# si220/Forest-SLAM

Measured on AMD Instinct MI355X. Metric: stereo frames/sec (extract+match+local-BA) at 600p, 1/8 MI355X; ATE RMSE, higher is better.
Workload: dtype mixed: u8/u16 integer (FAST, BRIEF, Hamming, SGM), f32 (ORB angle/Harris, back-projection), f64 (PnP, BA incl. its Schur GEMM on f64 MFMA); 1 GPU; stereo VO front end, configs[1]: 960x600, ORB nfeatures=1000, BF-Hamming xcheck (L+R), SGBM-3way 96 disp, back-projection, PnP-RANSAC, local BA K=10; width=960, height=600, nfeatures=1000, local_ba=window K=10 per frame, 10 LM iterations (fvo_ba_windows), parallelism=seq-per-gpu x1

## Files before the change

### forest-slam_amd/csrc/orb.hip

```cpp
#include <cmath>
#include <cstring>

#include "fvo_device.h"
#include "orb_pattern.inc"

namespace {

struct OrbDev {
  int nlevels, total_rows;
  int row0[FVO_MAX_LEVELS + 1];
  int w[FVO_MAX_LEVELS], h[FVO_MAX_LEVELS];
  long long off[FVO_MAX_LEVELS + 1];
  long long cand_off[FVO_MAX_LEVELS + 1];
  float scale[FVO_MAX_LEVELS];
  int nfeat[FVO_MAX_LEVELS];
  int tile0[FVO_MAX_LEVELS + 1];
  int ntx[FVO_MAX_LEVELS];
  int btile0[FVO_MAX_LEVELS + 1];
  int bntx[FVO_MAX_LEVELS];
};
__constant__ int c_umax[20];
__constant__ signed char c_pattern[256 * 4];

constexpr int kSelThreads = 512;
constexpr int kSelCap1 = 10000, kSelCap2 = 4096;

__device__ __forceinline__ int level_of_row(const OrbDev& G, int r) {
  int l = 0;
#pragma unroll
  for (int k = 1; k < FVO_MAX_LEVELS; ++k)
    if (k < G.nlevels && r >= G.row0[k]) l = k;
  return l;
}

__global__ void k_copy_level0(const uint8_t* __restrict__ img, int64_t stride, int pitch, uint8_t* __restrict__ pyr,
                              int64_t total, int W, int H) {
  int x = blockIdx.x * blockDim.x + threadIdx.x;
  int y = blockIdx.y;
  int b = blockIdx.z;
  if (x >= W) return;
  pyr[b * total + (int64_t)y * W + x] = img[b * stride + (int64_t)y * pitch + x];
}

__global__ void k_copy_level0_v(const uint4* __restrict__ img, int64_t stride16, int pitch16,
                                uint4* __restrict__ pyr, int64_t total16, int W16, int H, int batch) {
  const int64_t n = (int64_t)batch * H * W16;
  for (int64_t i = (int64_t)blockIdx.x * blockDim.x + threadIdx.x; i < n; i += (int64_t)gridDim.x * blockDim.x) {
    const int64_t row = i / W16;
    const int x = (int)(i - row * W16);
    const int b = (int)(row / H), y = (int)(row - (int64_t)b * H);
    pyr[b * total16 + (int64_t)y * W16 + x] = img[b * stride16 + (int64_t)y * pitch16 + x];
  }
}

constexpr int kResRows = 4, kResCols = 4;
__global__ void k_resize(const OrbDev G, uint8_t* __restrict__ pyr, int64_t total, int l, const int32_t* __restrict__ xofs,
                         const int32_t* __restrict__ xc1, const int32_t* __restrict__ yofs,
                         const int32_t* __restrict__ yc1) {
  const XcdBlock xb = xcd_block();
  const int x0 = (xb.x * blockDim.x + threadIdx.x) * kResCols;
  const int b = xb.z;
  const int w = G.w[l], h = G.h[l];
  if (x0 >= w) return;
  const int sw = G.w[l - 1], sh = G.h[l - 1];
  const uint8_t* src = pyr + b * total + G.off[l - 1];
  uint8_t* dst = pyr + b * total + G.off[l];
  int oxa[kResCols], oxb[kResCols];
  uint32_t cx0[kResCols], cx1[kResCols];
#pragma unroll
  for (int i = 0; i < kResCols; ++i) {
    const int ox = xofs[min(x0 + i, w - 1)];
    oxa[i] = ox >= 0 ? ox : (ox == -1 ? 0 : sw - 1);
    oxb[i] = ox >= 0 ? ox + 1 : oxa[i];
    cx1[i] = ox >= 0 ? (uint32_t)xc1[min(x0 + i, w - 1)] : 0u;
    cx0[i] = 256u - cx1[i];
  }
  const bool win8 = x0 + kResCols <= w && xofs[x0] >= 0 && xofs[x0 + kResCols - 1] >= 0 &&
                    oxb[kResCols - 1] - oxa[0] <= 7;
  auto window = [&](const uint8_t* row) -> uint64_t {
    const uintptr_t pa = reinterpret_cast<uintptr_t>(row + oxa[0]);
    const uint32_t* q = reinterpret_cast<const uint32_t*>(pa & ~(uintptr_t)3);
    const uint32_t sft = (uint32_t)(pa & 3);
    const uint32_t w0 = q[0], w1 = q[1], w2 = q[2];
    return ((uint64_t)__builtin_amdgcn_alignbyte(w2, w1, sft) << 32) | __builtin_amdgcn_alignbyte(w1, w0, sft);
  };
  uint32_t v[kResRows][kResCols];
#pragma unroll
  for (int k = 0; k < kResRows; ++k) {
    const int y = min(xb.y * kResRows + k, h - 1);
    const int oy = yofs[y];
    const int ra = oy >= 0 ? oy : (oy == -1 ? 0 : sh - 1), rb = oy >= 0 ? oy + 1 : ra;
    const uint32_t cy1 = oy >= 0 ? (uint32_t)yc1[y] : 0u, cy0 = 256u - cy1;
    const uint8_t* sa = src + (int64_t)ra * sw;
    const uint8_t* sb = src + (int64_t)rb * sw;
    if (win8) {
      const uint64_t wa = window(sa), wb = window(sb);
#pragma unroll
      for (int i = 0; i < kResCols; ++i) {
        const int da = 8 * (oxa[i] - oxa[0]), db = 8 * (oxb[i] - oxa[0]);
        const uint32_t ha = cx0[i] * (uint32_t)((wa >> da) & 255u) + cx1[i] * (uint32_t)((wa >> db) & 255u);
        const uint32_t hb = cx0[i] * (uint32_t)((wb >> da) & 255u) + cx1[i] * (uint32_t)((wb >> db) & 255u);
        v[k][i] = (ha * cy0 + hb * cy1 + 32768u) >> 16;
      }
    } else {
#pragma unroll
      for (int i = 0; i < kResCols; ++i) {
        const uint32_t ha = cx0[i] * sa[oxa[i]] + cx1[i] * sa[oxb[i]], hb = cx0[i] * sb[oxa[i]] + cx1[i] * sb[oxb[i]];
        v[k][i] = (ha * cy0 + hb * cy1 + 32768u) >> 16;
      }
    }
  }
#pragma unroll
  for (int k = 0; k < kResRows; ++k) {
    const int y = xb.y * kResRows + k;
#pragma unroll
    for (int i = 0; i < kResCols; ++i)
      if (y < h && x0 + i < w) dst[(int64_t)y * w + x0 + i] = (uint8_t)(v[k][i] > 255u ? 255u : v[k][i]);
  }
}

__constant__ int c_cdx[16] = {0, 1, 2, 3, 3, 3, 2, 1, 0, -1, -2, -3, -3, -3, -2, -1};
__constant__ int c_cdy[16] = {3, 3, 2, 1, 0, -1, -2, -3, -3, -3, -2, -1, 0, 1, 2, 3};

constexpr int kTW = 64, kTH = 32, kFT = 256;
static_assert(kTH <= 64 && kFT >= 2 * kTH && kFT % 64 == 0, "FAST tile shape");
constexpr int kRecKeep = 0, kRecPre = 8 * kTH, kRecSc = kRecPre + 2 * kTH;
constexpr int kTRec = kRecSc + kTH * kTW / 2;

constexpr int kFW = kTW + 2, kFH = kTH + 2;
constexpr int kPG = (kFW + 3) / 4;
constexpr int kIC = 4, kIW = kTW + 12, kIH = kTH + 8;

typedef unsigned short u16x2 __attribute__((ext_vector_type(2)));
__device__ __forceinline__ u16x2 as_u16x2(uint32_t v) { return __builtin_bit_cast(u16x2, v); }
__device__ __forceinline__ uint32_t as_u32(u16x2 v) { return __builtin_bit_cast(uint32_t, v); }
__device__ __forceinline__ u16x2 bytes02(uint32_t v) { return as_u16x2(__builtin_amdgcn_perm(0u, v, 0x0c020c00u)); }
__device__ __forceinline__ u16x2 bytes13(uint32_t v) { return as_u16x2(__builtin_amdgcn_perm(0u, v, 0x0c030c01u)); }

__device__ __forceinline__ u16x2 two_of_four(u16x2 a, u16x2 b, u16x2 c, u16x2 d) {
  const u16x2 lab = __builtin_elementwise_min(a, b), hab = __builtin_elementwise_max(a, b);
  const u16x2 lcd = __builtin_elementwise_min(c, d), hcd = __builtin_elementwise_max(c, d);
  return __builtin_elementwise_max(__builtin_elementwise_max(lab, lcd), __builtin_elementwise_min(hab, hcd));
}
__device__ __forceinline__ uint32_t fast_pre2(u16x2 v, u16x2 p0, u16x2 p4, u16x2 p8, u16x2 p12, u16x2 t) {
  const u16x2 vt = v + t, vm = __builtin_elementwise_sub_sat(v, t);
  auto br = [&](u16x2 p) { return __builtin_elementwise_sub_sat(p, vt); };
  auto dk = [&](u16x2 p) { return __builtin_elementwise_sub_sat(vm, p); };
  return as_u32(__builtin_elementwise_max(two_of_four(br(p0), br(p4), br(p8), br(p12)),
                                          two_of_four(dk(p0), dk(p4), dk(p8), dk(p12))));
}

__device__ __forceinline__ bool has9(unsigned m) {
  const unsigned mm = m | (m << 16);
  const unsigned c2 = mm & (mm >> 1), c4 = c2 & (c2 >> 2), c8 = c4 & (c4 >> 4), c9 = c8 & (c8 >> 1);
  return (c9 & 0xFFFFu) != 0;
}

__device__ __forceinline__ int tile_level(const OrbDev& G, int t) {
  int l = 0;
#pragma unroll
  for (int k = 1; k < FVO_MAX_LEVELS; ++k)
    if (k < G.nlevels && t >= G.tile0[k]) l = k;
  return l;
}

template <bool SCOREMAP>
__global__ __launch_bounds__(kFT) void k_fast_nms(const OrbDev G, const uint8_t* __restrict__ pyr,
                                                  uint8_t* __restrict__ score, uint8_t* __restrict__ trec,
                                                  int64_t total, int thr, int edge, int org, int ntiles) {
  __shared__ __attribute__((aligned(16))) uint8_t s_img[kIH][kIW];
  __shared__ __attribute__((aligned(16))) uint8_t s_sc[kFH][kFW];
  __shared__ uint16_t s_list[kFH * kFW];
  __shared__ uint16_t s_pre[kFH * kPG * 4];
  __shared__ uint32_t s_m[kTH][2];
  __shared__ int s_rp[kTH];
  __shared__ int s_n, s_npre;
  const XcdBlock xb = xcd_block();
  const int b = xb.y, t = xb.x;
  const int l = tile_level(G, t);
  const int lt = t - G.tile0[l];
  const int tx = lt % G.ntx[l], ty = lt / G.ntx[l];
  const int x0 = org + tx * kTW, y0 = org + ty * kTH;
  const int w = G.w[l], h = G.h[l];
  const uint8_t* im = pyr + b * total + G.off[l];
  if (x0 >= 8 && x0 + kTW + 12 <= w && y0 >= 4 && y0 + kTH + 4 <= h) {
    for (int i = threadIdx.x; i < kIH * (kIW / 4); i += kFT) {
      const int r = i / (kIW / 4), k = i % (kIW / 4);
      const uint8_t* p = im + (int64_t)(y0 - 4 + r) * w + x0 - 1 - kIC + 4 * k;
      const uint32_t* a = reinterpret_cast<const uint32_t*>(reinterpret_cast<uintptr_t>(p) & ~(uintptr_t)3);
      const uint32_t sh = (uint32_t)(reinterpret_cast<uintptr_t>(p) & 3);
      *reinterpret_cast<uint32_t*>(&s_img[r][4 * k]) = __builtin_amdgcn_alignbyte(a[1], a[0], sh);
    }
  } else {
    for (int i = threadIdx.x; i < kIH * kIW; i += kFT) {
      const int r = i / kIW, c = i % kIW;
      const int y = min(max(y0 - 4 + r, 0), h - 1), x = min(max(x0 - 1 - kIC + c, 0), w - 1);
      s_img[r][c] = im[(int64_t)y * w + x];
    }
  }
  for (int i = threadIdx.x; i < kFH * kFW / 4; i += kFT) reinterpret_cast<uint32_t*>(&s_sc[0][0])[i] = 0;
  if (threadIdx.x < 2 * kTH) (&s_m[0][0])[threadIdx.x] = 0u;
  if (threadIdx.x == 0) { s_n = 0; s_npre = 0; }
  __syncthreads();
  const u16x2 tt = {(unsigned short)thr, (unsigned short)thr};
  for (int i0 = 0; i0 < kFH * kPG; i0 += kFT) {
    const int i = i0 + threadIdx.x;
    const int r = i / kPG, g = i % kPG;
    const int y = y0 - 1 + r, xg = x0 - 1 + 4 * g;
    unsigned f = 0;
    if (i < kFH * kPG && y >= 3 && y < h - 3) {
      const uint32_t* rc = reinterpret_cast<const uint32_t*>(&s_img[r + 3][0]);
      const uint32_t dv = rc[g + 1];
      const uint32_t d0 = reinterpret_cast<const uint32_t*>(&s_img[r + 6][0])[g + 1];
      const uint32_t d8 = reinterpret_cast<const uint32_t*>(&s_img[r][0])[g + 1];
      const uint32_t d4 = __builtin_amdgcn_alignbyte(rc[g + 2], dv, 3);
      const uint32_t d12 = __builtin_amdgcn_alignbyte(dv, rc[g], 1);
      const uint32_t e = fast_pre2(bytes02(dv), bytes02(d0), bytes02(d4), bytes02(d8), bytes02(d12), tt);
      const uint32_t o = fast_pre2(bytes13(dv), bytes13(d0), bytes13(d4), bytes13(d8), bytes13(d12), tt);
      f = (unsigned)((e & 0xFFFFu) != 0) | (unsigned)((o & 0xFFFFu) != 0) << 1 | (unsigned)((e >> 16) != 0) << 2 |
          (unsigned)((o >> 16) != 0) << 3;
      const int lo = max(3 - xg, 0), hi = min(min(w - 3 - xg, kFW - 4 * g), 4);
      f &= hi > lo ? ((1u << hi) - 1u) & ~((1u << lo) - 1u) : 0u;
    }
    const unsigned long long m0 = __ballot(f & 1u), m1 = __ballot(f & 2u), m2 = __ballot(f & 4u),
                             m3 = __ballot(f & 8u);
    const int lane = threadIdx.x & 63;
    const unsigned long long below = (1ull << lane) - 1ull;
    int pos = __popcll(m0 & below) + __popcll(m1 & below) + __popcll(m2 & below) + __popcll(m3 & below);
    int base = 0;
    const int tot = __popcll(m0) + __popcll(m1) + __popcll(m2) + __popcll(m3);
    if (lane == 0 && tot) base = atomicAdd(&s_npre, tot);
    pos += __shfl(base, 0, 64);
    const int ib = r * kFW + 4 * g;
#pragma unroll
    for (int j = 0; j < 4; ++j)
      if ((f >> j) & 1u) s_pre[pos++] = (uint16_t)(ib + j);
  }
  __syncthreads();
  const int npre = s_npre;
  for (int j0 = 0; j0 < npre; j0 += kFT) {
    const int j = j0 + threadIdx.x;
    bool corner = false;
    int i = 0;
    if (j < npre) {
      i = s_pre[j];
      const int r = i / kFW, c = i % kFW;
      const int v = s_img[r + 3][c + kIC];
      const u16x2 vt = {(unsigned short)(v + thr), (unsigned short)(v + thr)};
      const u16x2 vm = {(unsigned short)(v - thr), (unsigned short)(v - thr)};
      uint32_t ab = 0, ad = 0;
#pragma unroll
      for (int k = 0; k < 8; ++k) {
        const uint32_t pk = (uint32_t)s_img[r + 3 + c_cdy[k]][c + kIC + c_cdx[k]] |
                            (uint32_t)s_img[r + 3 + c_cdy[k + 8]][c + kIC + c_cdx[k + 8]] << 16;
        const u16x2 sh = {(unsigned short)(15 - k), (unsigned short)(15 - k)};
        const uint32_t K = 0x10001u << k;
        ab |= as_u32((vt - as_u16x2(pk)) >> sh) & K;
        ad |= as_u32((as_u16x2(pk) - vm) >> sh) & K;
      }
      const unsigned bright = __builtin_amdgcn_perm(0u, ab, 0x0c0c0200u);
      const unsigned dark = __builtin_amdgcn_perm(0u, ad, 0x0c0c0200u);
      corner = has9(bright) || has9(dark);
    }
    const unsigned long long m = __ballot(corner);
    int base = 0;
    if ((threadIdx.x & 63) == 0 && m) base = atomicAdd(&s_n, __popcll(m));
    base = __shfl(base, 0, 64);
    if (corner) s_list[base + __popcll(m & ((1ull << (threadIdx.x & 63)) - 1ull))] = (uint16_t)i;
  }
  __syncthreads();
// ... 774 lines not shown
    g.scale[l] = s;
    g.w[l] = cv_round_f((float)c.width * inv);
    g.h[l] = cv_round_f((float)c.height * inv);
    g.off[l] = off;
    off += (int64_t)g.w[l] * g.h[l];
    g.row0[l] = row;
    row += g.h[l];
    int rw = std::max(g.w[l] - 2 * c.edge_threshold, 0), rh = std::max(g.h[l] - 2 * c.edge_threshold, 0);
    g.cand_off[l] = coff;
    coff += (int64_t)((rw + 1) / 2) * ((rh + 1) / 2) + 1;
  }
  g.off[c.nlevels] = off;
  g.row0[c.nlevels] = row;
  g.cand_off[c.nlevels] = coff;
  g.total_px = (off + 255) / 256 * 256;
  g.total_rows = row;
  g.cand_total = coff;
  {
    float factor = (float)(1.0 / sf);
    float nd = c.nfeatures * (1 - factor) / (1 - (float)std::pow((double)factor, (double)c.nlevels));
    int sum = 0;
    for (int l = 0; l < c.nlevels - 1; ++l) {
      g.nfeat[l] = cv_round_f(nd);
      sum += g.nfeat[l];
      nd *= factor;
    }
    g.nfeat[c.nlevels - 1] = std::max(c.nfeatures - sum, 0);
  }

  std::vector<int32_t> xo, xc, yo, yc;
  auto coeffs = [](int src, int dst, std::vector<int32_t>& ofs, std::vector<int32_t>& c1) {
    double inv_scale = (double)dst / (double)src;
    double scale = 1.0 / inv_scale;
    for (int d = 0; d < dst; ++d) {
      double fval = scale * ((double)d + 0.5) - 0.5;
      int ival = (int)std::floor(fval);
      if (ival >= 0 && src > 1) {
        if (ival < src - 1) {
          double frac = fval - (double)ival;
          ofs.push_back(ival);
          c1.push_back(frac < 0 ? 0 : (int)std::llrint(frac * 256.0));
        } else {
          ofs.push_back(-2);
          c1.push_back(0);
        }
      } else {
        ofs.push_back(-1);
        c1.push_back(0);
      }
    }
  };
  for (int l = 1; l < c.nlevels; ++l) {
    ctx->rt.xoff[l] = (int64_t)xo.size();
    coeffs(g.w[l - 1], g.w[l], xo, xc);
    ctx->rt.yoff[l] = (int64_t)yo.size();
    coeffs(g.h[l - 1], g.h[l], yo, yc);
  }
  if (xo.empty()) { xo.push_back(0); xc.push_back(0); yo.push_back(0); yc.push_back(0); }
  int rc = 0;
  if ((rc = fvo_alloc(ctx, &ctx->rt.xofs, xo.size())) || (rc = fvo_alloc(ctx, &ctx->rt.xc1, xc.size())) ||
      (rc = fvo_alloc(ctx, &ctx->rt.yofs, yo.size())) || (rc = fvo_alloc(ctx, &ctx->rt.yc1, yc.size())))
    return rc;
  FVO_HIP(ctx, hipMemcpy(ctx->rt.xofs, xo.data(), xo.size() * 4, hipMemcpyHostToDevice));
  FVO_HIP(ctx, hipMemcpy(ctx->rt.xc1, xc.data(), xc.size() * 4, hipMemcpyHostToDevice));
  FVO_HIP(ctx, hipMemcpy(ctx->rt.yofs, yo.data(), yo.size() * 4, hipMemcpyHostToDevice));
  FVO_HIP(ctx, hipMemcpy(ctx->rt.yc1, yc.data(), yc.size() * 4, hipMemcpyHostToDevice));

  int half = c.patch_size / 2;
  std::vector<int> umax(half + 2 > 20 ? half + 2 : 20, 0);
  int vmax = (int)std::floor(half * std::sqrt(2.f) / 2 + 1);
  int vmin = (int)std::ceil(half * std::sqrt(2.f) / 2);
  for (int v = 0; v <= vmax; ++v) umax[v] = (int)std::lrint(std::sqrt((double)half * half - v * v));
  for (int v = half, v0 = 0; v >= vmin; --v) {
    while (umax[v0] == umax[v0 + 1]) ++v0;
    umax[v] = v0;
    ++v0;
  }

  g.angle_pass = half > kAngR || c.edge_threshold < half;

  FVO_HIP(ctx, hipMemcpyToSymbol(HIP_SYMBOL(c_umax), umax.data(), sizeof(int) * 20));
  FVO_HIP(ctx, hipMemcpyToSymbol(HIP_SYMBOL(c_pattern), FVO_ORB_PATTERN, sizeof(FVO_ORB_PATTERN)));

  const int64_t B = c.max_batch;
  int64_t maxcand = 0;
  for (int l = 0; l < c.nlevels; ++l) maxcand = std::max<int64_t>(maxcand, g.cand_off[l + 1] - g.cand_off[l]);
  ctx->scratch_per = 2 * maxcand;
  if ((rc = fvo_alloc(ctx, &ctx->pyr, B * g.total_px)) ||
      (rc = fvo_alloc(ctx, &ctx->cand, B * g.cand_total)) ||
      (rc = fvo_alloc(ctx, &ctx->hel, B * g.cand_total)) || (rc = fvo_alloc(ctx, &ctx->ncand, B * c.nlevels)) ||
      (rc = fvo_alloc(ctx, &ctx->nsel1, B * c.nlevels)) || (rc = fvo_alloc(ctx, &ctx->nsel2, B * c.nlevels)) ||
      (rc = fvo_alloc(ctx, &ctx->koff, B * (c.nlevels + 1))) ||
      (rc = fvo_alloc(ctx, &ctx->scratch, B * c.nlevels * ctx->scratch_per)))
    return rc;
  if ((rc = fvo_alloc(ctx, &ctx->fast_rec, B * make_dev(g, c.edge_threshold).tile0[g.nlevels] * kTRec))) return rc;
  return 0;
}

namespace {
OrbDev make_dev(const OrbGeom& g, int org) {
  OrbDev G{};
  G.nlevels = g.nlevels;
  G.total_rows = g.total_rows;
  int t = 0, bt = 0;
  for (int l = 0; l < g.nlevels; ++l) {
    G.row0[l] = g.row0[l];
    G.w[l] = g.w[l];
    G.h[l] = g.h[l];
    G.off[l] = g.off[l];
    G.cand_off[l] = g.cand_off[l];
    G.scale[l] = g.scale[l];
    G.nfeat[l] = g.nfeat[l];
    const int ew = g.w[l] - 2 * org, eh = g.h[l] - 2 * org;
    G.ntx[l] = ew > 0 && eh > 0 ? (ew + kTW - 1) / kTW : 0;
    G.tile0[l] = t;
    t += G.ntx[l] ? G.ntx[l] * ((eh + kTH - 1) / kTH) : 0;
    G.bntx[l] = (g.w[l] + kBW - 1) / kBW;
    G.btile0[l] = bt;
    bt += G.bntx[l] * ((g.h[l] + kBH - 1) / kBH);
  }
  G.btile0[g.nlevels] = bt;
  G.row0[g.nlevels] = g.row0[g.nlevels];
  G.off[g.nlevels] = g.off[g.nlevels];
  G.cand_off[g.nlevels] = g.cand_off[g.nlevels];
  G.tile0[g.nlevels] = t;
  return G;
}
}

int orb_run(fvo_ctx* ctx, const uint8_t* images, int batch, int64_t image_stride, int pitch, float* kp, uint8_t* desc,
            int32_t* counts, int cap, hipStream_t s) {
  const fvo_config& c = ctx->cfg;
  const OrbGeom& g = ctx->g;
  const int L = g.nlevels;
  const int W = c.width, H = c.height;
  const int64_t total = g.total_px;
  const int thr = std::min(std::max(c.fast_threshold, 0), 255);
  const OrbDev G = make_dev(g, c.edge_threshold);
  const int ntiles = G.tile0[L];
  const bool vec = ((uintptr_t)images & 15) == 0 && (image_stride & 15) == 0 && (pitch & 15) == 0 && (W & 15) == 0 &&
                   (total & 15) == 0;
  if (vec) {
    const int64_t n16 = (int64_t)batch * H * (W / 16);
    const int nblk = (int)std::min<int64_t>((n16 + 255) / 256, 4096);
    FVO_TIMED(ctx, KN_ORB_COPY, s, hipLaunchKernelGGL(k_copy_level0_v, dim3(nblk), dim3(256), 0, s,
                                                      reinterpret_cast<const uint4*>(images), image_stride / 16,
                                                      pitch / 16, reinterpret_cast<uint4*>(ctx->pyr), total / 16, W / 16,
                                                      H, batch));
  } else {
    FVO_TIMED(ctx, KN_ORB_COPY, s, hipLaunchKernelGGL(k_copy_level0, dim3((W + 255) / 256, H, batch), dim3(256), 0, s,
                                                      images, image_stride, pitch, ctx->pyr, total, W, H));
  }
  for (int l = 1; l < L; ++l)
    FVO_TIMED(ctx, KN_ORB_RESIZE, s, hipLaunchKernelGGL(k_resize, dim3((g.w[l] + 256 * kResCols - 1) / (256 * kResCols), (g.h[l] + kResRows - 1) / kResRows, batch), dim3(256), 0, s, G, ctx->pyr, total, l,
                       ctx->rt.xofs + ctx->rt.xoff[l], ctx->rt.xc1 + ctx->rt.xoff[l], ctx->rt.yofs + ctx->rt.yoff[l],
                       ctx->rt.yc1 + ctx->rt.yoff[l]));
  if (ntiles > 0)
    FVO_TIMED(ctx, KN_ORB_FAST, s, hipLaunchKernelGGL(k_fast_nms<false>, dim3(ntiles, batch), dim3(kFT), 0, s, G, ctx->pyr,
                       nullptr, ctx->fast_rec, total, thr, c.edge_threshold, c.edge_threshold, ntiles));
  FVO_TIMED(ctx, KN_ORB_SELECT1, s, hipLaunchKernelGGL(HIP_KERNEL_NAME(k_select<ElemFast, kSelCap1, true>), dim3(batch, L),
                     dim3(kSelThreads), 0, s, G, ctx->fast_rec, ntiles, c.edge_threshold, ctx->cand, ctx->ncand,
                     ctx->nsel1, ctx->scratch, ctx->scratch_per, g.cand_total, L, 2));
  FVO_TIMED(ctx, KN_ORB_HARRIS, s, hipLaunchKernelGGL(k_harris, dim3(32, L, batch), dim3(256), 0, s, G, ctx->pyr, ctx->cand, ctx->nsel1, ctx->hel, total,
                     g.cand_total, L));
  FVO_TIMED(ctx, KN_ORB_SELECT2, s, hipLaunchKernelGGL(HIP_KERNEL_NAME(k_select<ElemHarris, kSelCap2, false>), dim3(batch, L),
                     dim3(kSelThreads), 0, s, G, nullptr, ntiles, c.edge_threshold, ctx->hel, ctx->nsel1,
                     ctx->nsel2, ctx->scratch, ctx->scratch_per, g.cand_total, L, 1));
  FVO_TIMED(ctx, KN_ORB_OFFSETS, s, hipLaunchKernelGGL(k_offsets, dim3((batch + 63) / 64), dim3(64), 0, s, ctx->nsel2, ctx->koff, counts, batch, L, cap));
  if (g.angle_pass) {
    FVO_TIMED(ctx, KN_ORB_ANGLE, s, hipLaunchKernelGGL(k_angle, dim3(16, L, batch), dim3(256), 0, s, G, ctx->pyr, ctx->hel, ctx->nsel2, ctx->koff, kp,
                       total, g.cand_total, L, cap, c.patch_size));
    FVO_TIMED(ctx, KN_ORB_BRIEF, s, hipLaunchKernelGGL(k_brief<false>, dim3(64, batch), dim3(256), 0, s, G, ctx->pyr, ctx->hel, ctx->koff, kp, counts,
                       desc, total, g.cand_total, L, cap, c.patch_size));
  } else {
    FVO_TIMED(ctx, KN_ORB_BRIEF, s, hipLaunchKernelGGL(k_brief<true>, dim3(64, batch), dim3(256), 0, s, G, ctx->pyr, ctx->hel, ctx->koff, kp, counts,
                       desc, total, g.cand_total, L, cap, c.patch_size));
  }
  ctx->orb_last_batch = batch;
  FVO_LAUNCH_CHECK(ctx);
  return 0;
}

int orb_blur_debug(fvo_ctx* ctx) {
  const OrbGeom& g = ctx->g;
  if (!ctx->blur) {
    int rc = fvo_alloc(ctx, &ctx->blur, (int64_t)ctx->cfg.max_batch * g.total_px);
    if (rc) return rc;
  }
  if (ctx->orb_last_batch > 0) {
    const OrbDev G = make_dev(g, 0);
    hipLaunchKernelGGL(k_blur, dim3(G.btile0[g.nlevels], ctx->orb_last_batch), dim3(256), 0, 0, G, ctx->pyr, ctx->blur,
                       g.total_px);
    FVO_LAUNCH_CHECK(ctx);
  }
  FVO_HIP(ctx, hipDeviceSynchronize());
  return 0;
}

int orb_score_debug(fvo_ctx* ctx) {
  const OrbGeom& g = ctx->g;
  if (!ctx->score) {
    int rc = fvo_alloc(ctx, &ctx->score, (int64_t)ctx->cfg.max_batch * g.total_px);
    if (rc) return rc;
  }
  if (ctx->orb_last_batch > 0) {
    const OrbDev G = make_dev(g, 0);
    const int ntiles = G.tile0[g.nlevels];
    hipLaunchKernelGGL(k_fast_nms<true>, dim3(ntiles, ctx->orb_last_batch), dim3(kFT), 0, 0, G, ctx->pyr, ctx->score,
                       nullptr, g.total_px, std::min(std::max(ctx->cfg.fast_threshold, 0), 255),
                       ctx->cfg.edge_threshold, 0, ntiles);
    FVO_LAUNCH_CHECK(ctx);
  }
  FVO_HIP(ctx, hipDeviceSynchronize());
  return 0;
}

namespace {
__global__ void k_pack_keys(const float* __restrict__ k, uint64_t* __restrict__ a, int n) {
  int i = blockIdx.x * blockDim.x + threadIdx.x;
  if (i < n) a[i] = ((uint64_t)__float_as_uint(k[i]) << 32) | (uint32_t)i;
}
__global__ void k_unpack_idx(const uint64_t* __restrict__ a, int32_t* __restrict__ idx, int n) {
  int i = blockIdx.x * blockDim.x + threadIdx.x;
  if (i < n) idx[i] = (int32_t)(uint32_t)a[i];
}
__global__ __launch_bounds__(kSelThreads) void k_select_test(uint64_t* __restrict__ a, int n, int keep,
                                                             int32_t* __restrict__ scratch, int32_t* __restrict__ out_n) {
  __shared__ SelShared sh;
  int r = select_block<ElemHarris>(sh, a, n, keep, scratch, scratch + n);
  if (threadIdx.x == 0) *out_n = r;
}
}

int orb_retain_best_run(fvo_ctx* ctx, const float* keys, int n, int keep, int32_t* idx_out, int32_t* n_out,
                         hipStream_t s) {
  uint64_t* a = nullptr;
  int32_t* scr = nullptr;
  FVO_HIP(ctx, hipMallocAsync((void**)&a, sizeof(uint64_t) * (size_t)std::max(n, 1), s));
  FVO_HIP(ctx, hipMallocAsync((void**)&scr, sizeof(int32_t) * 2 * (size_t)std::max(n, 1), s));
  hipLaunchKernelGGL(k_pack_keys, dim3((n + 255) / 256 + 1), dim3(256), 0, s, keys, a, n);
  hipLaunchKernelGGL(k_select_test, dim3(1), dim3(kSelThreads), 0, s, a, n, keep, scr, n_out);
  hipLaunchKernelGGL(k_unpack_idx, dim3((n + 255) / 256 + 1), dim3(256), 0, s, a, idx_out, n);
  FVO_HIP(ctx, hipFreeAsync(a, s));
  FVO_HIP(ctx, hipFreeAsync(scr, s));
  FVO_LAUNCH_CHECK(ctx);
  return 0;
}
```

### forest-slam_amd/csrc/sgbm.hip

```cpp
#include <algorithm>
#include <cstdlib>
#include <type_traits>

#include "fvo_device.h"
#include "sgbm_params.h"

namespace {

typedef unsigned short u16x2 __attribute__((ext_vector_type(2)));

__device__ __forceinline__ u16x2 as_v(uint32_t x) { return __builtin_bit_cast(u16x2, x); }
__device__ __forceinline__ uint32_t as_u(u16x2 v) { return __builtin_bit_cast(uint32_t, v); }
__device__ __forceinline__ u16x2 vmin(u16x2 a, u16x2 b) { return __builtin_elementwise_min(a, b); }
__device__ __forceinline__ u16x2 splat(uint32_t s) { return as_v((s & 0xFFFFu) | (s << 16)); }
__device__ __forceinline__ u16x2 splat_p2(uint32_t m, uint32_t P2) { return as_v(__umul24(m, 0x10001u) + P2 * 0x10001u); }

constexpr uint32_t kSent = 0x7FFFu;

constexpr int kQPrev = 0x90;
constexpr int kQNext = 0xF9;
constexpr int kQX1 = 0xB1;
constexpr int kQX2 = 0x4E;

template <int CTRL>
// ... 742 lines not shown
  if constexpr (!S2) return;

  const int nseg = (W1 + SEG - 1) / SEG;
  uint32_t Rst[PQ];
  uint32_t minR = 0;
#pragma unroll
  for (int k = 0; k < PQ; ++k) Rst[k] = 0;
  uint32_t Vn[SEG][PQ], Pn[SEG][PQ], Mn[SEG], ckn[CKW];
  auto ldck = [&](int sg) {
    const int slot = SEG * (sg + 1) > W1 - 1 ? nck - 1 : sg;
    const uint32_t* cp = ckptr(slot);
#pragma unroll
    for (int kk = 0; kk < CKW; kk += 4) {
      const uint4 w4 = *reinterpret_cast<const uint4*>(cp + kk);
      ckn[kk] = w4.x; ckn[kk + 1] = w4.y; ckn[kk + 2] = w4.z; ckn[kk + 3] = w4.w;
    }
  };
  auto ldcol = [&](int sg, int i) {
    const int xx = max(W1 - 1 - (SEG * sg + i), 0);
    ld(xx, Vn[i]);
    ldp(xx, Pn[i]);
    Mn[i] = ldm(xx);
  };
  auto ldseg = [&](int sg) {
    ldck(sg);
#pragma unroll
    for (int i = SEG - 1; i >= 0; --i) ldcol(sg, i);
  };
  ldseg(0);
  auto ihi_of = [&](int sg) { return min(SEG - 1, W1 - 1 - SEG * sg); };
  uint32_t wk = 0, wn = 0;
  auto wta = [&](int i, const uint32_t* Sw) {
    uint32_t kmin = 0;
#pragma unroll
    for (int kk = 0; kk < PQ; ++kk) {
      const uint32_t jj = (uint32_t)(2 * kk) | ((uint32_t)(2 * kk + 1) << 8);
      const uint32_t klo = __builtin_amdgcn_perm(Sw[kk], jj, 0x0c050400u);
      const uint32_t khi = __builtin_amdgcn_perm(Sw[kk], jj, 0x0c070601u);
      kmin = kk == 0 ? min(klo, khi) : min(kmin, min(klo, khi));
    }
    kmin += (uint32_t)(q * DQ);
    kmin = dmin<kQX1>(kmin);
    kmin = dmin<kQX2>(kmin);
    kmin = dmin<kRHalfMirror>(kmin);
    kmin = dmin<kRMirror>(kmin);
    const int d = (int)(kmin & 0xFFu);
    uint32_t* sw = reinterpret_cast<uint32_t*>(&s_S[r][q * DQ]);
#pragma unroll
    for (int kk = 0; kk < PQ; ++kk) sw[kk] = Sw[kk];
    asm volatile("" ::: "memory");
    const uint32_t nb = ((uint32_t)s_S[r][max(d - 1, 0)] << 16) | s_S[r][min(d + 1, D - 1)];
    asm volatile("" ::: "memory");
    wk = q == i ? kmin : wk;
    wn = q == i ? nb : wn;
  };
  auto segment = [&](int sg, auto full_t) {
    constexpr bool FULL = decltype(full_t)::value;
    if constexpr (FULL) {
      uint32_t lst[PQ], Cs[SEG][PQ], part[SEG][PQ];
#pragma unroll
      for (int kk = 0; kk < PQ; ++kk) lst[kk] = ckn[kk];
      uint32_t lmin = ckn[PQ];
      ldck(sg + 1);
#pragma unroll
      for (int t = 0; t < SEG; ++t) {
        const int a = SEG - 1 - t, c = t;
        if (t < SEG / 2) {
          derive16<PQ>(Pn[a], Vn[a], Cs[a], Mn[a], P1, p.P2, q);
          derive16<PQ>(Pn[c], Vn[c], Cs[c], Mn[c], P1, p.P2, q);
        }
        lmin = step16<PQ>(lst, Cs[a], q, P1, lmin, p.P2);
        minR = step16<PQ>(Rst, Cs[c], q, P1, minR, p.P2);
        if (t < SEG / 2) {
#pragma unroll
          for (int kk = 0; kk < PQ; ++kk) {
            part[a][kk] = as_u(as_v(lst[kk]) + as_v(Vn[a][kk]));
            part[c][kk] = as_u(as_v(Rst[kk]) + as_v(Vn[c][kk]));
          }
        } else {
          uint32_t Sa[PQ], Sc[PQ];
#pragma unroll
          for (int kk = 0; kk < PQ; ++kk) {
            Sa[kk] = as_u(as_v(part[a][kk]) + as_v(lst[kk]));
            Sc[kk] = as_u(as_v(part[c][kk]) + as_v(Rst[kk]));
          }
          wta(a, Sa);
          wta(c, Sc);
          const int u = t - SEG / 2;
          ldcol(sg + 1, SEG - 1 - u);
          ldcol(sg + 1, u);
        }
      }
    } else {
      uint32_t lst[PQ], Ls[SEG][PQ], Cs[SEG][PQ];
      const bool zero = SEG * (sg + 1) > W1 - 1;
#pragma unroll
      for (int kk = 0; kk < PQ; ++kk) lst[kk] = zero ? 0u : ckn[kk];
      uint32_t lmin = zero ? 0u : ckn[PQ];
#pragma unroll
      for (int i = SEG - 1; i >= 0; --i) {
        derive16<PQ>(Pn[i], Vn[i], Cs[i], Mn[i], P1, p.P2, q);
        if (i <= ihi_of(sg)) lmin = step16<PQ>(lst, Cs[i], q, P1, lmin, p.P2);
#pragma unroll
        for (int kk = 0; kk < PQ; ++kk) Ls[i][kk] = as_u(as_v(lst[kk]) + as_v(Vn[i][kk]));
      }
#pragma unroll
      for (int i = 0; i < SEG; ++i) {
        if (i > ihi_of(sg)) break;
        minR = step16<PQ>(Rst, Cs[i], q, P1, minR, p.P2);
        uint32_t Sw[PQ];
#pragma unroll
        for (int kk = 0; kk < PQ; ++kk) Sw[kk] = as_u(as_v(Ls[i][kk]) + as_v(Rst[kk]));
        wta(i, Sw);
      }
    }
    {
      const int ihi = FULL ? SEG - 1 : ihi_of(sg);
      {
        const bool colv = q < SEG && q <= ihi;
        const int x1 = W1 - 1 - (SEG * sg + q);
        if (colv) key[(x1 + p.minX1 - p.minD - (D - 1)) & (RK - 1)] = 0xFFFFFFFFu;
        if (colv) {
          const int best = (int)(wk >> 8), d = (int)(wk & 0xFFu);
          const int sm1 = (int)(wn >> 16), sp1 = (int)(wn & 0xFFFFu);
          const int x2 = x1 + p.minX1 - d - p.minD;
          if (x2 >= 0 && x2 < W && best < 0x7FFF)
            atomicMin(&key[x2 & (RK - 1)], ((uint32_t)best << 16) | (uint32_t)(0xFFFF - x1));
          int dd;
          if (0 < d && d < D - 1) {
            const int denom2 = max(sm1 + sp1 - 2 * best, 1);
            dd = d * 16 + ((sm1 - sp1) * 16 + denom2) / (denom2 * 2);
          } else {
            dd = d * 16;
          }
          sraw[x1 & (RS - 1)] = (int16_t)(dd + p.minD * 16);
        }
      }
      const int x1_lo = W1 - 1 - (SEG * sg + ihi);
      {
        const int cnt = ihi >= 0 ? min(next_chk - (x1_lo + D) + 1, SEG) : 0;
        const bool act = q < cnt && rowok;
        const int d1 = checked(next_chk - q);
        *(act ? out + (next_chk - q + p.minX1) : sink) = (int16_t)d1;
        if (cnt > 0) next_chk -= cnt;
      }
    }
  };
#pragma unroll 1
  for (int sg = 0; sg < nseg - 1; ++sg) segment(sg, std::true_type{});
  segment(nseg - 1, std::false_type{});
  for (int x1 = next_chk - q; x1 >= 0; x1 -= 16) check(x1);
}

__global__ void k_sg_median(const int16_t* __restrict__ raw, int16_t* __restrict__ out, int W, int H,
                            const uint32_t* __restrict__ fail, int16_t invalid, int32_t* __restrict__ status) {
  const int x = blockIdx.x * blockDim.x + threadIdx.x, y = blockIdx.y, b = blockIdx.z;
  if (status && x == 0 && y == 0) status[b] = (fail && fail[b]) ? FVO_SGBM_HANDOFF_TIMEOUT : FVO_SGBM_OK;
  if (x >= W) return;
  const int16_t* s = raw + (int64_t)b * W * H;
  int v[9];
  int k = 0;
#pragma unroll
  for (int dy = -1; dy <= 1; ++dy)
#pragma unroll
    for (int dx = -1; dx <= 1; ++dx) {
      const int yy = min(max(y + dy, 0), H - 1), xx = min(max(x + dx, 0), W - 1);
      v[k++] = s[(int64_t)yy * W + xx];
    }
#define SG_S(a, b) { int t_ = min(v[a], v[b]); v[b] = max(v[a], v[b]); v[a] = t_; }
  SG_S(1, 2) SG_S(4, 5) SG_S(7, 8) SG_S(0, 1) SG_S(3, 4) SG_S(6, 7) SG_S(1, 2) SG_S(4, 5) SG_S(7, 8)
  SG_S(0, 3) SG_S(5, 8) SG_S(4, 7) SG_S(3, 6) SG_S(1, 4) SG_S(2, 5) SG_S(4, 7) SG_S(4, 2) SG_S(6, 4)
  SG_S(4, 2)
#undef SG_S
  out[((int64_t)b * H + y) * W + x] = (fail && fail[b]) ? invalid : (int16_t)v[4];
}

__global__ void k_sg_prep(uint32_t* ctl, int nb) {
  const int t = threadIdx.x;
  if (t == 0) {
    ctl[0] = 0;
    const uint32_t g = ctl[1] + 1;
    ctl[1] = g >= (1u << 25) ? 1u : g;
  }
  for (int b = t; b < nb; b += blockDim.x) ctl[4 + b] = 0;
}

int sg_nck(const SgParams& p) { return p.width1 / 8 + 2; }
int sg_ckw(int D) { return D / 32 + 1 <= 4 ? 4 : 8; }
int sg_nblk(const SgParams& p) { return (p.H + 3) / 4; }

template <int D>
void launch_sgbm(fvo_ctx* ctx, const SgParams& p, const uint8_t* L, const uint8_t* R, int nb, int64_t stride,
                 int pitch, int16_t* disp, int32_t* status, hipStream_t s) {
  uint16_t* V = ctx->sg_V;
  uint16_t* M = ctx->sg_M;
  const int nck = sg_nck(p);
  const int16_t invalid = (int16_t)((p.minD - 1) * 16);
  const fvo_config& cfg = ctx->cfg;
  if (cfg.sgbm_mode == FVO_SGBM_CLASSIC) {
    const int g = sg_lanes(cfg), cbr = sg_cols(cfg);
    typedef void (*CostKernel)(const uint8_t*, const uint8_t*, int64_t, int, SgParams, uint16_t*, uint16_t*, SgLink);
    CostKernel kern;
    int gg, cb;
    if (g == 16) kern = k_sg_costvert<D, 32, 16, false>, gg = 16, cb = 32;
    else if (g == 4 && cbr == 32) kern = k_sg_costvert<D, 32, 4, false>, gg = 4, cb = 32;
    else if (g == 4) kern = k_sg_costvert<D, 64, 4, false>, gg = 4, cb = 64;
    else if (cbr == 16) kern = k_sg_costvert<D, 16, 8, false>, gg = 8, cb = 16;
    else kern = k_sg_costvert<D, 32, 8, false>, gg = 8, cb = 32;
    const dim3 gcv((p.width1 + cb - 1) / cb, p.nstripes, nb);
    const SgLink lk{};
    FVO_TIMED(ctx, KN_SG_VERT, s, hipLaunchKernelGGL(kern, gcv, dim3(gg * cb), 0, s, L, R, stride, pitch, p, V, M, lk));
    FVO_TIMED(ctx, KN_SG_ROWS, s, hipLaunchKernelGGL(HIP_KERNEL_NAME(k_sg_rows<D, kSwBoth>), dim3(sg_nblk(p), nb), dim3(64), 0, s,
                                                     V, M, p, ctx->sg_ckpt, nck, ctx->sg_raw));
    FVO_TIMED(ctx, KN_SG_MEDIAN, s, hipLaunchKernelGGL(k_sg_median, dim3((p.W + 255) / 256, p.H, nb), dim3(256), 0, s,
                                                       ctx->sg_raw, disp, p.W, p.H, nullptr, invalid, status));
    return;
  }
  const int nk = sg_nk(p);
  const int64_t us = cfg.sgbm_handoff_us > 0 ? cfg.sgbm_handoff_us : 250000;
  const SgLink lk{ctx->sg_ckpt, nck, nk, ctx->sg_hand, ctx->sg_ctl, (uint64_t)us * 100u, cfg.sgbm_handoff_us < 0 ? 1 : 0};
  hipLaunchKernelGGL(k_sg_prep, dim3(1), dim3(256), 0, s, ctx->sg_ctl, nb);
  FVO_TIMED(ctx, KN_SG_VERT, s, hipLaunchKernelGGL(HIP_KERNEL_NAME(k_sg_costvert<D, kSgCB, 8, true>),
                                                   dim3(nk * p.nstripes * nb), dim3(8 * kSgCB), 0, s, L, R, stride, pitch,
                                                   p, V, M, lk));
  FVO_TIMED(ctx, KN_SG_ROWS, s, hipLaunchKernelGGL(HIP_KERNEL_NAME(k_sg_rows<D, kSwRight>), dim3(sg_nblk(p), nb), dim3(64), 0, s,
                                                   V, M, p, ctx->sg_ckpt, nck, ctx->sg_raw));
  FVO_TIMED(ctx, KN_SG_MEDIAN, s, hipLaunchKernelGGL(k_sg_median, dim3((p.W + 255) / 256, p.H, nb), dim3(256), 0, s,
                                                     ctx->sg_raw, disp, p.W, p.H, ctx->sg_ctl + 4, invalid, status));
}

}

int sgbm_init(fvo_ctx* ctx) {
  const fvo_config& c = ctx->cfg;
  SgParams p = make_params(c);
  const int64_t B = c.sgbm_max_batch > 0 ? std::min(c.sgbm_max_batch, c.max_batch) : c.max_batch;
  const int64_t plane = (int64_t)p.width1 * p.D;
  int rc;
  const int64_t vol = (int64_t)(p.HG4 + p.nstripes) * 4 * plane;
  const int64_t ckp = (int64_t)sg_nblk(p) * sg_nck(p) * 64 * sg_ckw(p.D);
  const int64_t hand = (int64_t)p.H * 2 * (p.D / 32) * 16;
  if ((rc = fvo_alloc(ctx, &ctx->sg_V, B * vol)) || (rc = fvo_alloc(ctx, &ctx->sg_M, B * vol / p.D)) ||
      (rc = fvo_alloc(ctx, &ctx->sg_ckpt, B * ckp)) ||
      (rc = fvo_alloc(ctx, &ctx->sg_raw, B * p.H * p.W)) || (rc = fvo_alloc(ctx, &ctx->sg_hand, B * hand)) ||
      (rc = fvo_alloc(ctx, &ctx->sg_ctl, 4 + B)))
    return rc;
  FVO_HIP(ctx, hipMemset(ctx->sg_hand, 0, B * hand * sizeof(uint64_t)));
  FVO_HIP(ctx, hipMemset(ctx->sg_ctl, 0, (4 + B) * sizeof(uint32_t)));
  return 0;
}

int sgbm_run(fvo_ctx* ctx, const uint8_t* L, const uint8_t* R, int batch, int64_t image_stride, int pitch,
             int16_t* disp, int32_t* status, hipStream_t s) {
  SgParams p = make_params(ctx->cfg);
  switch (p.D) {
    case 64: launch_sgbm<64>(ctx, p, L, R, batch, image_stride, pitch, disp, status, s); break;
    case 96: launch_sgbm<96>(ctx, p, L, R, batch, image_stride, pitch, disp, status, s); break;
    default: launch_sgbm<128>(ctx, p, L, R, batch, image_stride, pitch, disp, status, s); break;
  }
  FVO_LAUNCH_CHECK(ctx);
  return 0;
}
```

Before: 5914 frames/s.

## Tile pyramid resize through LDS and vectorize SGBM 3x3 median

The ORB pyramid resize now stages each 128x64 output tile's source window into LDS with 16-byte loads. It computes horizontal taps with perm+udot2, reuses the horizontal result when consecutive output rows share a source row, and writes dword-packed outputs using a lane shuffle. It falls back to the old direct path when the tile's source window does not fit. Separately, the SGBM median filter now handles 8 columns by 4 rows per thread using packed 16-bit min/max and 16-byte loads and stores, sharing the column sorts between rows. Both changes aim to cut per-pixel memory traffic and instruction count, at the cost of more complex alignment and edge handling.

New measurement: 5974 frames/s (median of 6 runs). 1.01x the previous value.

```diff
diff --git a/forest-slam_amd/csrc/orb.hip b/forest-slam_amd/csrc/orb.hip
--- a/forest-slam_amd/csrc/orb.hip
+++ b/forest-slam_amd/csrc/orb.hip
@@ -53,18 +53,12 @@
   }
 }
 
-constexpr int kResRows = 4, kResCols = 4;
-__global__ void k_resize(const OrbDev G, uint8_t* __restrict__ pyr, int64_t total, int l, const int32_t* __restrict__ xofs,
-                         const int32_t* __restrict__ xc1, const int32_t* __restrict__ yofs,
-                         const int32_t* __restrict__ yc1) {
-  const XcdBlock xb = xcd_block();
-  const int x0 = (xb.x * blockDim.x + threadIdx.x) * kResCols;
-  const int b = xb.z;
-  const int w = G.w[l], h = G.h[l];
+constexpr int kResCols = 4;
+__device__ __forceinline__ void resize_direct(const uint8_t* __restrict__ src, uint8_t* __restrict__ dst, int w, int h,
+                                              int sw, int sh, int x0, int y0, int rows, const int32_t* __restrict__ xofs,
+                                              const int32_t* __restrict__ xc1, const int32_t* __restrict__ yofs,
+                                              const int32_t* __restrict__ yc1) {
   if (x0 >= w) return;
-  const int sw = G.w[l - 1], sh = G.h[l - 1];
-  const uint8_t* src = pyr + b * total + G.off[l - 1];
-  uint8_t* dst = pyr + b * total + G.off[l];
   int oxa[kResCols], oxb[kResCols];
   uint32_t cx0[kResCols], cx1[kResCols];
 #pragma unroll
@@ -84,10 +78,9 @@
     const uint32_t w0 = q[0], w1 = q[1], w2 = q[2];
     return ((uint64_t)__builtin_amdgcn_alignbyte(w2, w1, sft) << 32) | __builtin_amdgcn_alignbyte(w1, w0, sft);
   };
-  uint32_t v[kResRows][kResCols];
-#pragma unroll
-  for (int k = 0; k < kResRows; ++k) {
-    const int y = min(xb.y * kResRows + k, h - 1);
+#pragma unroll 1
+  for (int y = y0; y < min(y0 + rows, h); ++y) {
+    uint32_t v[kResCols];
     const int oy = yofs[y];
     const int ra = oy >= 0 ? oy : (oy == -1 ? 0 : sh - 1), rb = oy >= 0 ? oy + 1 : ra;
     const uint32_t cy1 = oy >= 0 ? (uint32_t)yc1[y] : 0u, cy0 = 256u - cy1;
@@ -100,22 +93,142 @@
         const int da = 8 * (oxa[i] - oxa[0]), db = 8 * (oxb[i] - oxa[0]);
         const uint32_t ha = cx0[i] * (uint32_t)((wa >> da) & 255u) + cx1[i] * (uint32_t)((wa >> db) & 255u);
         const uint32_t hb = cx0[i] * (uint32_t)((wb >> da) & 255u) + cx1[i] * (uint32_t)((wb >> db) & 255u);
-        v[k][i] = (ha * cy0 + hb * cy1 + 32768u) >> 16;
+        v[i] = (ha * cy0 + hb * cy1 + 32768u) >> 16;
       }
     } else {
 #pragma unroll
       for (int i = 0; i < kResCols; ++i) {
         const uint32_t ha = cx0[i] * sa[oxa[i]] + cx1[i] * sa[oxb[i]], hb = cx0[i] * sb[oxa[i]] + cx1[i] * sb[oxb[i]];
-        v[k][i] = (ha * cy0 + hb * cy1 + 32768u) >> 16;
-      }
-    }
-  }
-#pragma unroll
-  for (int k = 0; k < kResRows; ++k) {
-    const int y = xb.y * kResRows + k;
+        v[i] = (ha * cy0 + hb * cy1 + 32768u) >> 16;
+      }
+    }
 #pragma unroll
     for (int i = 0; i < kResCols; ++i)
-      if (y < h && x0 + i < w) dst[(int64_t)y * w + x0 + i] = (uint8_t)(v[k][i] > 255u ? 255u : v[k][i]);
+      if (x0 + i < w) dst[(int64_t)y * w + x0 + i] = (uint8_t)(v[i] > 255u ? 255u : v[i]);
+  }
+}
+
+constexpr int kRzTW = 128, kRzTH = 64, kRzSR = 8;
+constexpr int kRzLds = 1024;
+static_assert(kRzTW == 32 * kResCols && kRzTH == 8 * kRzSR, "resize tile shape");
+__global__ __launch_bounds__(256) void k_resize(const OrbDev G, uint8_t* __restrict__ pyr, int64_t total, int l,
+                                                const int32_t* __restrict__ xofs, const int32_t* __restrict__ xc1,
+                                                const int32_t* __restrict__ yofs, const int32_t* __restrict__ yc1) {
+  __shared__ uint4 s_src[kRzLds + 1];
+  const int tid = threadIdx.x, cg = tid & 31, strip = tid >> 5;
+  const int tx0 = blockIdx.x * kRzTW, ty0 = blockIdx.y * kRzTH, b = blockIdx.z;
+  const int w = G.w[l], h = G.h[l], sw = G.w[l - 1], sh = G.h[l - 1];
+  uint8_t* img = pyr + b * total;
+  const int tw = min(kRzTW, w - tx0), th = min(kRzTH, h - ty0);
+  auto first = [](int o, int n) { return o >= 0 ? o : (o == -1 ? 0 : n - 1); };
+  auto last = [](int o, int n) { return o >= 0 ? o + 1 : (o == -1 ? 0 : n - 1); };
+  const int c0 = first(xofs[tx0], sw), c1 = last(xofs[tx0 + tw - 1], sw);
+  const int r0 = first(yofs[ty0], sh), r1 = last(yofs[ty0 + th - 1], sh);
+  const int ncols = c1 - c0 + 1, nrows = r1 - r0 + 1;
+  const int pitch16 = (ncols + 15 + 15) >> 4;
+  const int x0 = tx0 + cg * kResCols;
+  int wofs = 0, span = 0;
+  uint32_t sel[kResCols], cxw[kResCols];
+#pragma unroll
+  for (int i = 0; i < kResCols; ++i) {
+    const int x = min(x0 + i, w - 1);
+    const int ox = xofs[x], oa = first(ox, sw), ob = last(ox, sw);
+    const uint32_t c = ox >= 0 ? (uint32_t)xc1[x] : 0u;
+    if (i == 0) wofs = oa;
+    span = ob - wofs;
+    sel[i] = 0x0c000c00u | (uint32_t)(oa - wofs) | ((uint32_t)(ob - wofs) << 16);
+    cxw[i] = (256u - c) | (c << 16);
+  }
+  if (!__syncthreads_and(span <= 7) || pitch16 * nrows > kRzLds) {
+    resize_direct(img + G.off[l - 1], img + G.off[l], w, h, sw, sh, x0, ty0 + strip * kRzSR, kRzSR, xofs, xc1, yofs, yc1);
+    return;
+  }
+  wofs -= c0;
+
+  uint32_t rinfo[kRzSR];
+#pragma unroll
+  for (int k = 0; k < kRzSR; ++k) {
+    const int yc = min(ty0 + strip * kRzSR + k, h - 1), oy = yofs[yc];
+    rinfo[k] = (uint32_t)(first(oy, sh) - r0) | ((uint32_t)(last(oy, sh) - first(oy, sh)) << 10) |
+               ((oy >= 0 ? (uint32_t)yc1[yc] : 0u) << 16);
+  }
+  const int64_t g0 = G.off[l - 1] + (int64_t)r0 * sw + c0;
+  uint4 stage[kRzLds / 256];
+#pragma unroll
+  for (int k = 0; k < kRzLds / 256; ++k) {
+    const int i = tid + 256 * k, rr = i / pitch16, j = i - rr * pitch16;
+    const int64_t ga = g0 + (int64_t)rr * sw;
+    const int nblk = (((int)ga & 15) + ncols + 15) >> 4;
+    const bool ok = rr < nrows && j < nblk;
+    stage[k] = reinterpret_cast<const uint4*>(img + ((ok ? ga : g0) & ~(int64_t)15))[ok ? j : 0];
+  }
+#pragma unroll
+  for (int k = 0; k < kRzLds / 256; ++k)
+    if (tid + 256 * k < nrows * pitch16) s_src[tid + 256 * k] = stage[k];
+  __syncthreads();
+
+  typedef unsigned short us2 __attribute__((ext_vector_type(2)));
+  const uint32_t* lds = reinterpret_cast<const uint32_t*>(s_src);
+  const int g0lo = (int)g0 & 15;
+  auto hrow = [&](int rr, uint32_t (&hv)[kResCols]) {
+    const uint32_t p = (uint32_t)(rr * pitch16 * 16 + ((g0lo + rr * sw) & 15) + wofs);
+    const uint32_t* q = lds + (p >> 2);
+    const uint32_t w0 = q[0], w1 = q[1], w2 = q[2], sft = p & 3;
+    const uint32_t lo = __builtin_amdgcn_alignbyte(w1, w0, sft), hi = __builtin_amdgcn_alignbyte(w2, w1, sft);
+#pragma unroll
+    for (int i = 0; i < kResCols; ++i)
+      hv[i] = __builtin_amdgcn_udot2(__builtin_bit_cast(us2, __builtin_amdgcn_perm(hi, lo, sel[i])),
+                                     __builtin_bit_cast(us2, cxw[i]), 0u, false);
+  };
+  uint8_t* dst = img + G.off[l] + tx0;
+  uint32_t hp[kResCols] = {};
+  int prb = -1;
+#pragma unroll
+  for (int k = 0; k < kRzSR; ++k) {
+    const int y = ty0 + strip * kRzSR + k;
+    const int ra = (int)(rinfo[k] & 1023u), rb = ra + (int)((rinfo[k] >> 10) & 1u);
+    const uint32_t cy = rinfo[k] >> 16, cyw = (256u - cy) | (cy << 16);
+    uint32_t ha[kResCols], hb[kResCols], acc[kResCols];
+    if (ra == prb) {
+#pragma unroll
+      for (int i = 0; i < kResCols; ++i) ha[i] = hp[i];
+    } else {
+      hrow(ra, ha);
+    }
+    if (rb == ra) {
+#pragma unroll
+      for (int i = 0; i < kResCols; ++i) hb[i] = ha[i];
+    } else {
+      hrow(rb, hb);
+    }
+    prb = rb;
+#pragma unroll
+    for (int i = 0; i < kResCols; ++i) {
+      hp[i] = hb[i];
+      acc[i] = min(__builtin_amdgcn_udot2(__builtin_bit_cast(us2, ha[i] | (hb[i] << 16)), __builtin_bit_cast(us2, cyw),
+                                          32768u, false), 0xFFFFFFu);
+    }
+    const uint32_t own = __builtin_amdgcn_perm(__builtin_amdgcn_perm(acc[3], acc[2], 0x0c0c0602u),
+                                               __builtin_amdgcn_perm(acc[1], acc[0], 0x0c0c0602u), 0x05040100u);
+    const uint32_t prev = __shfl_up(own, 1, 32);
+    const int a = (int)((G.off[l] + (int64_t)y * w + tx0) & 3);
+    const uint32_t dw = (uint32_t)((((uint64_t)own << 32) | prev) >> (8 * (4 - a)));
+    if (y < h) {
+      uint8_t* row = dst + (int64_t)y * w;
+      const int cd = cg * kResCols - a;
+      if (cd >= 0 && cd + 3 < tw) {
+        *reinterpret_cast<uint32_t*>(row + cd) = dw;
+      } else {
+#pragma unroll
+        for (int j = 0; j < 4; ++j)
+          if (cd + j >= 0 && cd + j < tw) row[cd + j] = (uint8_t)(dw >> (8 * j));
+      }
+      if (cg == 31) {
+#pragma unroll
+        for (int j = 0; j < 3; ++j)
+          if (j < a && cd + 4 + j < tw) row[cd + 4 + j] = (uint8_t)(own >> (8 * (4 - a + j)));
+      }
+    }
   }
 }
 
@@ -1196,7 +1309,7 @@
                                                       images, image_stride, pitch, ctx->pyr, total, W, H));
   }
   for (int l = 1; l < L; ++l)
-    FVO_TIMED(ctx, KN_ORB_RESIZE, s, hipLaunchKernelGGL(k_resize, dim3((g.w[l] + 256 * kResCols - 1) / (256 * kResCols), (g.h[l] + kResRows - 1) / kResRows, batch), dim3(256), 0, s, G, ctx->pyr, total, l,
+    FVO_TIMED(ctx, KN_ORB_RESIZE, s, hipLaunchKernelGGL(k_resize, dim3((g.w[l] + kRzTW - 1) / kRzTW, (g.h[l] + kRzTH - 1) / kRzTH, batch), dim3(256), 0, s, G, ctx->pyr, total, l,
                        ctx->rt.xofs + ctx->rt.xoff[l], ctx->rt.xc1 + ctx->rt.xoff[l], ctx->rt.yofs + ctx->rt.yoff[l],
                        ctx->rt.yc1 + ctx->rt.yoff[l]));
   if (ntiles > 0)
diff --git a/forest-slam_amd/csrc/sgbm.hip b/forest-slam_amd/csrc/sgbm.hip
--- a/forest-slam_amd/csrc/sgbm.hip
+++ b/forest-slam_amd/csrc/sgbm.hip
@@ -918,9 +918,66 @@
   for (int x1 = next_chk - q; x1 >= 0; x1 -= 16) check(x1);
 }
 
-__global__ void k_sg_median(const int16_t* __restrict__ raw, int16_t* __restrict__ out, int W, int H,
-                            const uint32_t* __restrict__ fail, int16_t invalid, int32_t* __restrict__ status) {
-  const int x = blockIdx.x * blockDim.x + threadIdx.x, y = blockIdx.y, b = blockIdx.z;
+typedef short sg_s2 __attribute__((ext_vector_type(2)));
+constexpr int kMedRows = 4;
+__host__ __device__ inline bool sg_median_vec(const void* raw, const void* out, int W) {
+  return W % 8 == 0 && (((uintptr_t)raw | (uintptr_t)out) & 15) == 0;
+}
+inline dim3 sg_median_grid(const void* raw, const void* out, int W, int H, int nb) {
+  if (sg_median_vec(raw, out, W)) return dim3(((W / 8) * ((H + kMedRows - 1) / kMedRows) + 255) / 256, 1, nb);
+  return dim3((W + 255) / 256, H, nb);
+}
+
+#define SG_PK(a, b) { const sg_s2 t_ = __builtin_elementwise_min(a, b); b = __builtin_elementwise_max(a, b); a = t_; }
+__device__ __forceinline__ void sg_median_rows8(const int16_t* __restrict__ s, int16_t* __restrict__ o, int W, int H,
+                                                int x0, int y0, bool bad, int16_t invalid) {
+  sg_s2 t[kMedRows + 2][4][3];
+#pragma unroll
+  for (int k = 0; k < kMedRows + 2; ++k) {
+    const int16_t* row = s + (int64_t)min(max(y0 - 1 + k, 0), H - 1) * W;
+    const uint4 c4 = *reinterpret_cast<const uint4*>(row + x0);
+    const uint32_t c[4] = {c4.x, c4.y, c4.z, c4.w};
+    const uint32_t l = (uint16_t)row[max(x0 - 1, 0)], r = (uint16_t)row[min(x0 + 8, W - 1)];
+#pragma unroll
+    for (int j = 0; j < 4; ++j) {
+      const uint32_t lo = j ? (c[j - 1] >> 16) | (c[j] << 16) : l | (c[0] << 16);
+      const uint32_t hi = j < 3 ? (c[j] >> 16) | (c[j + 1] << 16) : (c[3] >> 16) | (r << 16);
+      sg_s2 a = __builtin_bit_cast(sg_s2, lo), m = __builtin_bit_cast(sg_s2, c[j]), z = __builtin_bit_cast(sg_s2, hi);
+      SG_PK(m, z) SG_PK(a, m) SG_PK(m, z)
+      t[k][j][0] = a, t[k][j][1] = m, t[k][j][2] = z;
+    }
+  }
+  const uint32_t inv2 = (uint16_t)invalid * 0x10001u;
+#pragma unroll
+  for (int k = 0; k < kMedRows; ++k) {
+    uint32_t res[4];
+#pragma unroll
+    for (int j = 0; j < 4; ++j) {
+      sg_s2 v0 = t[k][j][0], v1 = t[k][j][1], v2 = t[k][j][2], v3 = t[k + 1][j][0], v4 = t[k + 1][j][1],
+            v5 = t[k + 1][j][2], v6 = t[k + 2][j][0], v7 = t[k + 2][j][1], v8 = t[k + 2][j][2];
+      SG_PK(v0, v3) SG_PK(v5, v8) SG_PK(v4, v7) SG_PK(v3, v6) SG_PK(v1, v4) SG_PK(v2, v5) SG_PK(v4, v7) SG_PK(v4, v2)
+      SG_PK(v6, v4) SG_PK(v4, v2)
+      res[j] = bad ? inv2 : __builtin_bit_cast(uint32_t, v4);
+    }
+    if (y0 + k < H) *reinterpret_cast<uint4*>(o + (int64_t)(y0 + k) * W + x0) = make_uint4(res[0], res[1], res[2], res[3]);
+  }
+}
+#undef SG_PK
+
+__global__ __launch_bounds__(256) void k_sg_median(const int16_t* __restrict__ raw, int16_t* __restrict__ out, int W, int H,
+                                                   const uint32_t* __restrict__ fail, int16_t invalid,
+                                                   int32_t* __restrict__ status) {
+  const int b = blockIdx.z;
+  if (sg_median_vec(raw, out, W)) {
+    const int W8 = W >> 3, i = blockIdx.x * blockDim.x + threadIdx.x;
+    const bool bad = fail && fail[b];
+    if (status && i == 0) status[b] = bad ? FVO_SGBM_HANDOFF_TIMEOUT : FVO_SGBM_OK;
+    const int yg = i / W8;
+    if (yg * kMedRows >= H) return;
+    sg_median_rows8(raw + (int64_t)b * W * H, out + (int64_t)b * W * H, W, H, (i - yg * W8) * 8, yg * kMedRows, bad, invalid);
+    return;
+  }
+  const int x = blockIdx.x * blockDim.x + threadIdx.x, y = blockIdx.y;
   if (status && x == 0 && y == 0) status[b] = (fail && fail[b]) ? FVO_SGBM_HANDOFF_TIMEOUT : FVO_SGBM_OK;
   if (x >= W) return;
   const int16_t* s = raw + (int64_t)b * W * H;
@@ -978,7 +1035,7 @@
     FVO_TIMED(ctx, KN_SG_VERT, s, hipLaunchKernelGGL(kern, gcv, dim3(gg * cb), 0, s, L, R, stride, pitch, p, V, M, lk));
     FVO_TIMED(ctx, KN_SG_ROWS, s, hipLaunchKernelGGL(HIP_KERNEL_NAME(k_sg_rows<D, kSwBoth>), dim3(sg_nblk(p), nb), dim3(64), 0, s,
                                                      V, M, p, ctx->sg_ckpt, nck, ctx->sg_raw));
-    FVO_TIMED(ctx, KN_SG_MEDIAN, s, hipLaunchKernelGGL(k_sg_median, dim3((p.W + 255) / 256, p.H, nb), dim3(256), 0, s,
+    FVO_TIMED(ctx, KN_SG_MEDIAN, s, hipLaunchKernelGGL(k_sg_median, sg_median_grid(ctx->sg_raw, disp, p.W, p.H, nb), dim3(256), 0, s,
                                                        ctx->sg_raw, disp, p.W, p.H, nullptr, invalid, status));
     return;
   }
@@ -991,7 +1048,7 @@
                                                    p, V, M, lk));
   FVO_TIMED(ctx, KN_SG_ROWS, s, hipLaunchKernelGGL(HIP_KERNEL_NAME(k_sg_rows<D, kSwRight>), dim3(sg_nblk(p), nb), dim3(64), 0, s,
                                                    V, M, p, ctx->sg_ckpt, nck, ctx->sg_raw));
-  FVO_TIMED(ctx, KN_SG_MEDIAN, s, hipLaunchKernelGGL(k_sg_median, dim3((p.W + 255) / 256, p.H, nb), dim3(256), 0, s,
+  FVO_TIMED(ctx, KN_SG_MEDIAN, s, hipLaunchKernelGGL(k_sg_median, sg_median_grid(ctx->sg_raw, disp, p.W, p.H, nb), dim3(256), 0, s,
                                                      ctx->sg_raw, disp, p.W, p.H, ctx->sg_ctl + 4, invalid, status));
 }
 
```
